# OpenMatchmaking/microservice-matchmaking

Measured on NVIDIA H100. Metric: matches/sec, higher is better.
Workload: dtype int32/u64

## Files before the change

### microservice-matchmaking_b200/csrc/mm_common.cuh

```cuda
#pragma once
#include <cuda_runtime.h>
#include <stdint.h>

#include "../../include/mm_engine.h"

namespace mm {

constexpr int kBlock = 512;
constexpr uint32_t kTile = 2048;
constexpr uint32_t kMaxRows = 2048;
constexpr uint32_t kMaxStages = 4;
constexpr uint32_t kTileBytes = kTile * (8 + 2);
constexpr uint32_t kMaxSegs = MM_MAX_GROUPS * MM_MAX_MODES;
constexpr uint32_t kChunkHist = 256;
constexpr uint32_t kFastBins = 255;
constexpr uint64_t kEmptyKey = 0xFFFFFFFFFFFFFFFFull;
constexpr uint64_t kTombKey = 0xFFFFFFFFFFFFFFFEull;
constexpr uint64_t kFreeVal = 0xFFFFFFFFFFFFFFFFull;
constexpr uint64_t kPending = 0x8000000000000000ull;
constexpr uint32_t kGenMask = 0x7FFFFFFFu;

struct PoolView {
  uint64_t* id;
  int32_t* rating;
  uint8_t* mode;
  uint8_t* tsize;
  uint32_t* ts;
  uint16_t* bin;
  uint32_t* seq;
};
struct PoolMeta {
  uint32_t* fill;
  uint32_t* chunk_tab;
  uint32_t* bump;
  uint32_t* tot;
  uint32_t* chist;
  uint32_t max_ch;
};
// ... 252 lines not shown
```

### microservice-matchmaking_b200/csrc/mm_engine.cu

```cuda
#include <cuda_runtime.h>

#include <algorithm>
#include <cstdio>
#include <cstdlib>
#include <cstring>
#include <mutex>
#include <new>
#include <vector>

#include "mm_kernels.cuh"
#include "mm_stats.cuh"

using namespace mm;

namespace {

struct Pool {
  PoolView v{};
  PoolMeta m{};
  uint32_t n = 0;
};

struct Table {
  unsigned long long* kv = nullptr;
// ... 38 lines not shown
  Pool pool[2];
  int cur = 0;
  uint32_t gen = 1;
  uint32_t seq_next = 0;
  Pool snap;
  uint32_t snap_gen = 0, snap_seq = 0;
  bool has_snap = false;

  bool use_active = true, dense_ids = false;
  uint64_t hcap = 0;
  Table tab[2];
  int tcur = 0;
  uint64_t n_active = 0, n_tomb = 0;

  uint32_t R = 0;
  uint32_t helpers = 0;
  int rows_per_sm = 2;
  int rank_impl = 3;
  uint32_t place_stages = 0;
  int fused_ok = 0;
  int tick_impl = 1;
  size_t tick_smem = 0;
  uint32_t *d_M = nullptr, *d_P = nullptr;
  uint32_t *d_outbase = nullptr, *d_binlim = nullptr;
  uint16_t* d_bin_key = nullptr;
  int32_t max_spread = -1;
  SegInfo* d_seg = nullptr;
  uint32_t* d_left_bits = nullptr;
  uint64_t* d_members = nullptr;
  uint32_t* d_members32 = nullptr;
  uint32_t* d_members32_alt = nullptr;
  mm_lobby_hdr* d_hdr_alt = nullptr;
  uint32_t* d_src_idx = nullptr;
  mm_lobby_hdr* d_hdr = nullptr;
  uint32_t* d_emit_seq = nullptr;
  uint32_t max_lobbies = 0;
  uint32_t* d_rescnt = nullptr;
  TickCtr* d_ctr2 = nullptr;
  TickCtr* d_ctr = nullptr;
  int ctr_idx = 0;
  TickCtr* h_ctr = nullptr;

  uint32_t enq_cap = 0;
  uint64_t *d_in_id = nullptr, *d_hslot = nullptr;
  int32_t* d_in_rating = nullptr;
  uint8_t *d_in_mode = nullptr, *d_code = nullptr;
// ... 237 lines not shown
  CK(cudaMemcpy(e->d_lut, lut.data(), e->KR * 2, cudaMemcpyHostToDevice));
  CK(cudaMemcpy(e->d_grp_lut, grp.data(), e->KR, cudaMemcpyHostToDevice));
  CK(cudaMemcpy(e->d_mode_tsize, tsz.data(), MM_MAX_MODES, cudaMemcpyHostToDevice));
  CK(cudaMemcpy(e->d_seg_bin_lo, seg_lo.data(), (e->n_segs + 1) * 4, cudaMemcpyHostToDevice));
  CK(cudaMemcpy(e->d_seg_L, seg_L.data(), e->n_segs * 4, cudaMemcpyHostToDevice));
  return MM_OK;
}

BinMap bin_map(const mm_engine* e) {
  BinMap b{};
  b.lut = e->d_lut; b.key_lo = e->key_lo; b.KR = e->KR; b.stride = e->stride; b.K = e->K;
  return b;
}

int alloc_tick_scratch(mm_engine* e) {
  uint32_t total = (uint32_t)e->n_sms * (uint32_t)e->rows_per_sm;
  if (total > kMaxRows) total = kMaxRows;
  e->helpers = total >= 64 ? 4u : (total > 1 ? 1u : 0u);
  e->R = total - e->helpers;
  if (e->d_M) { cudaFree(e->d_M); cudaFree(e->d_P); cudaFree(e->d_rescnt); }
  CK(cudaMalloc(&e->d_M, (size_t)(e->R + 1) * e->Kp * 4));
  CK(cudaMalloc(&e->d_P, (size_t)(e->R + 1) * e->Kp * 4));
  CK(cudaMalloc(&e->d_rescnt, (size_t)(e->R + 1) * 4));
  return MM_OK;
}

int ensure_enq_scratch(mm_engine* e, uint32_t n) {
  if (n <= e->enq_cap) return MM_OK;
  cudaFree(e->d_in_id); cudaFree(e->d_hslot); cudaFree(e->d_in_rating); cudaFree(e->d_in_mode);
  cudaFree(e->d_code); cudaFree(e->d_in_ts); cudaFree(e->d_blocksum); cudaFree(e->d_part); cudaFree(e->d_in_key);
  cudaFree(e->d_in_handle);
  e->enq_cap = 0;
  const size_t c = (size_t)n + 64;
  CK(cudaMalloc(&e->d_in_id, c * 8));
  CK(cudaMalloc(&e->d_hslot, c * 8));
  CK(cudaMalloc(&e->d_in_rating, c * 4));
  CK(cudaMalloc(&e->d_in_mode, c));
  CK(cudaMalloc(&e->d_code, c));
  CK(cudaMalloc(&e->d_part, c * 2));
  CK(cudaMalloc(&e->d_in_key, c * 2));
  CK(cudaMalloc(&e->d_in_handle, c * 4));
  CK(cudaMalloc(&e->d_in_ts, c * 4));
  CK(cudaMalloc(&e->d_blocksum, (std::min<size_t>(c, kEnqChunkDev) / 256 + 2) * 4));
  e->enq_cap = n;
  return MM_OK;
}
// ... 80 lines not shown

TailArgs tail_args(mm_engine* e) {
  TailArgs t{};
  t.Kp = e->Kp; t.K = e->K; t.n_segs = e->n_segs; t.max_spread = e->max_spread; t.layout = tail_layout(e);
  t.tot = e->pool[e->cur].m.tot; t.seg_bin_lo = e->d_seg_bin_lo; t.seg_L = e->d_seg_L; t.bin_seg = e->d_bin_seg;
  t.n_cut = e->n_cut; t.part_cut = e->d_part_cut; t.cut_lp_lo = e->d_cut_lp_lo;
  t.bin_key = e->d_bin_key; t.outbase = e->d_outbase; t.binlim = e->d_binlim; t.seg = e->d_seg; t.ctr = e->d_ctr;
  t.fill = e->pool[e->cur].m.fill;
  t.dst = e->pool[e->cur ^ 1].m;
  return t;
}
uint32_t tick_rows(const mm_engine* e) {
  const uint64_t tiles = (uint64_t)e->pool[e->cur].n / kTile + e->n_segs;
  const uint32_t total = e->R + e->helpers;
  const uint32_t want = std::min(32u, std::max(e->helpers, (total * 14 / 100 + e->min_L - 1) / e->min_L));
  return (uint32_t)std::min<uint64_t>(total - want, std::max<uint64_t>(1, (tiles + 1) / 2));
}

PlaceArgs place_args(mm_engine* e, bool want_seq) {
  const Pool& p = e->pool[e->cur];
  PlaceArgs a{};
  a.bins16 = p.v.bin; a.ids = p.v.id; a.meta = p.m;
  a.K = e->K; a.Kp = e->Kp; a.R = tick_rows(e); a.stages = e->place_stages; a.fast_ok = e->rank_impl == 3; a.max_nb = e->max_nb;
  a.seg_bin_lo = e->d_seg_bin_lo; a.bin_seg = e->d_bin_seg; a.M = e->d_M; a.P = e->d_P;
  a.outbase = e->d_outbase; a.binlim = e->d_binlim; a.members = e->d_members;
  a.src_idx = want_seq ? e->d_src_idx : nullptr;
  a.left_bits = e->d_left_bits; a.rescnt = e->d_rescnt; a.ctr = e->d_ctr;
  return a;
}
uint32_t next_gen(const mm_engine* e) { return e->gen >= kGenMask ? 1u : e->gen + 1; }
EpiArgs epi_args(mm_engine* e, bool want_seq, bool headers) {
  EpiArgs a{};
  a.src = e->pool[e->cur].v; a.dst = e->pool[e->cur ^ 1].v;
  a.src_meta = e->pool[e->cur].m; a.dst_meta = e->pool[e->cur ^ 1].m;
  a.R = tick_rows(e); a.new_gen = next_gen(e); a.n_segs = e->n_segs; a.n_groups = e->cfg.n_groups; a.Kp = e->Kp;
  a.write_headers = headers ? 1u : 0u;
  a.rescnt = e->d_rescnt; a.left_bits = e->d_left_bits; a.act = act_view(e); a.seg = e->d_seg; a.seg_L = e->d_seg_L; a.part_cut = e->d_part_cut;
  a.seg_bin_lo = e->d_seg_bin_lo;
  a.hdr = e->d_hdr; a.src_idx = want_seq ? e->d_src_idx : nullptr; a.emit_seq = want_seq ? e->d_emit_seq : nullptr;
  a.ctr = e->d_ctr;
  return a;
}

int tick_phase_a(mm_engine* e) {
  const Pool& p = e->pool[e->cur];
  CK(cudaMemsetAsync(e->d_ctr, 0, sizeof(TickCtr), e->stream));
  CK(cudaEventRecord(e->ev[0], e->stream));
  const uint32_t rows = tick_rows(e);
  k_hist<512><<<rows, 512, hist_smem_bytes(e->max_nb), e->stream>>>(p.v.bin, p.m, e->n_segs, rows, e->Kp, e->max_nb, e->d_seg_bin_lo, e->d_M);
  CK(cudaEventRecord(e->ev[1], e->stream));
  k_colscan<<<(e->K + 31) / 32 + 1, kScanBlock, colscan_smem(e), e->stream>>>(rows, e->d_M, e->d_P, tail_args(e));
  CK(cudaGetLastError());
  return MM_OK;
}

int tick_phase_b(mm_engine* e, bool want_seq) {
  CK(cudaEventRecord(e->ev[2], e->stream));
  const uint32_t rows = tick_rows(e);
  k_place<512><<<rows, 512, place_smem_bytes(e->max_nb, e->place_stages), e->stream>>>(place_args(e, want_seq),
                                                                                  e->pool[e->cur].m.fill, e->n_segs);
  CK(cudaEventRecord(e->ev[3], e->stream));
  if (e->pool[e->cur ^ 1].m.chist)
    CK(cudaMemsetAsync(e->pool[e->cur ^ 1].m.chist, 0, (size_t)e->n_chunks * kChunkHist * 4, e->stream));
  k_epilogue<512><<<std::max<uint32_t>(1, std::min<uint32_t>((uint32_t)e->n_sms, 2 * rows)), 512, 0, e->stream>>>(epi_args(e, want_seq, true));
  CK(cudaGetLastError());
  CK(cudaEventRecord(e->ev[4], e->stream));
  CK(cudaMemcpyAsync(e->h_ctr, e->d_ctr, sizeof(TickCtr), cudaMemcpyDeviceToHost, e->stream));
  CK(cudaStreamSynchronize(e->stream));
  return MM_OK;
}

bool use_fused(const mm_engine* e) { return e->tick_impl == 1 && e->fused_ok; }
// ... 18 lines not shown
  CK(cudaEventRecord(e->ev[4], e->stream));
  CK(cudaMemcpyAsync(e->h_ctr, e->d_ctr, sizeof(TickCtr), cudaMemcpyDeviceToHost, e->stream));
  CK(cudaStreamSynchronize(e->stream));
  return MM_OK;
}

int tick_commit(mm_engine* e, uint32_t n, mm_tick_stats* stats) {
  const TickCtr& c = *e->h_ctr;
  mm_tick_stats st{};
  st.pool_before = n; st.n_lobbies = c.n_lobbies; st.n_matched = c.n_matched; st.n_residual = c.n_resid;
  st.n_dead = c.n_dead; st.n_launches = 4;
  float ms = 0;
  CK(cudaEventElapsedTime(&ms, e->ev[0], e->ev[4]));
  st.device_us = ms * 1000.f;
  if (e->last_fused) {
    st.n_launches = 1;
    st.hist_us = (float)(c.t[1] - c.t[0]) * 1e-3f;
    st.scan_us = (float)(c.t[2] - c.t[1]) * 1e-3f;
    st.place_us = (float)(c.t[3] - c.t[2]) * 1e-3f;
    st.epilogue_us = (float)(c.t[6] - c.t[3]) * 1e-3f;
    if (std::getenv("MM_TRACE")) {
      const double us = 1e3 / ((double)e->clock_khz * tick_rows(e));
      std::fprintf(stderr, "[mm] t0=0 rows_p1_done=%.1f tail_done=%.1f bar1=%.1f place_start=%.1f rows_place_done=%.1f bar2=%.1f end=%.1f us"
                   " | place stall/row hand full empty loop: h0 %.1f %.1f %.1f %.1f h1 %.1f %.1f %.1f %.1f us\n",
                   (c.t[8] - c.t[0]) * 1e-3, (c.t[5] - c.t[0]) * 1e-3, (c.t[1] - c.t[0]) * 1e-3, (c.t[2] - c.t[0]) * 1e-3,
                   (c.t[10] - c.t[0]) * 1e-3, (c.t[3] - c.t[0]) * 1e-3, (c.t[6] - c.t[0]) * 1e-3,
                   c.stall[0][0] * us, c.stall[0][1] * us, c.stall[0][2] * us, c.stall[0][3] * us,
                   c.stall[1][0] * us, c.stall[1][1] * us, c.stall[1][2] * us, c.stall[1][3] * us);
    }
  } else {
    CK(cudaEventElapsedTime(&ms, e->ev[0], e->ev[1]));
    st.hist_us = ms * 1000.f;
    CK(cudaEventElapsedTime(&ms, e->ev[1], e->ev[2]));
    st.scan_us = ms * 1000.f;
    CK(cudaEventElapsedTime(&ms, e->ev[2], e->ev[3]));
    st.place_us = ms * 1000.f;
    CK(cudaEventElapsedTime(&ms, e->ev[3], e->ev[4]));
    st.epilogue_us = ms * 1000.f;
  }
  e->gen = next_gen(e);
  e->cur ^= 1;
  e->pool[e->cur].n = c.n_resid;
  e->match_valid = true;
  e->match_n = n;
  e->last = st;
  if (stats) *stats = st;
  if (c.chist_bad) {
    std::snprintf(e->last_err, sizeof(e->last_err), "%u placement tiles disagree with their chunk histograms", c.chist_bad);
    return MM_E_STATE;
  }
  return MM_OK;
// ... 122 lines not shown
  e->cfg = *cfg;
  e->device = cfg->device;
  e->capacity = cfg->capacity;
  e->use_active = !(cfg->flags & MM_F_NO_DEDUPE);
  e->dense_ids = e->use_active && (cfg->flags & MM_F_DENSE_IDS);
  auto bail = [&](int code) { mm_destroy(e); return code; };
  if (cudaSetDevice(e->device) != cudaSuccess) return bail(MM_E_CUDA);
  cudaDeviceProp prop{};
  if (cudaGetDeviceProperties(&prop, e->device) != cudaSuccess) return bail(MM_E_CUDA);
  e->n_sms = prop.multiProcessorCount;
  if (cudaDeviceGetAttribute(&e->clock_khz, cudaDevAttrClockRate, e->device) != cudaSuccess) return bail(MM_E_CUDA);
  e->smem_optin = prop.sharedMemPerBlockOptin;
  e->smem_sm = prop.sharedMemPerMultiprocessor;
  if (cudaStreamCreateWithFlags(&e->stream, cudaStreamNonBlocking) != cudaSuccess) return bail(MM_E_CUDA);
  if (cudaStreamCreateWithFlags(&e->d2h_stream, cudaStreamNonBlocking) != cudaSuccess) return bail(MM_E_CUDA);
  if (cudaStreamCreateWithFlags(&e->copy_stream, cudaStreamNonBlocking) != cudaSuccess ||
      cudaEventCreateWithFlags(&e->ev_copy, cudaEventDisableTiming) != cudaSuccess)
    return bail(MM_E_CUDA);
  for (auto& ev : e->ev)
    if (cudaEventCreate(&ev) != cudaSuccess) return bail(MM_E_CUDA);
  if ((rc = build_tables(e))) return bail(rc);
  {
    const size_t static_smem = sizeof(Geo) + 512;
    const uint32_t st_max = 2;
    for (uint32_t st = st_max; st >= 2 && !e->place_stages; --st)
      if (2 * (place_smem_bytes(e->max_nb, st) + static_smem + 1024) <= e->smem_sm) { e->place_stages = st; e->rows_per_sm = 2; }
    for (uint32_t st = kMaxStages; st >= 1 && !e->place_stages; --st)
      if (place_smem_bytes(e->max_nb, st) + static_smem + 1024 <= e->smem_optin) { e->place_stages = st; e->rows_per_sm = 1; }
    if (!e->place_stages || colscan_smem(e) + static_smem + 1024 > e->smem_optin) {
      std::snprintf(e->last_err, sizeof(e->last_err), "key domain too large for shared memory: %u bins", e->Kp);
      return bail(MM_E_ARG);
    }
    bool ok = allow_max_smem(e, k_colscan) == cudaSuccess && allow_max_smem(e, k_hist<512>) == cudaSuccess &&
              allow_max_smem(e, k_place<512>) == cudaSuccess && allow_max_smem(e, k_tick<512>) == cudaSuccess;
    if (!ok) return bail(fail(e, cudaGetLastError(), "cudaFuncSetAttribute"));
  }
  e->n_chunks = (e->capacity + kTile - 1) / kTile + e->n_segs + 2;
  if ((uint64_t)e->n_chunks * e->n_segs * 4 > (8ull << 30)) return bail(MM_E_CAP);
  if ((rc = alloc_pool(e, e->pool[0])) || (rc = alloc_pool(e, e->pool[1]))) return bail(rc);
  if (cudaMalloc(&e->d_left_bits, (pool_slots(e) / 32 + 64) * 4) != cudaSuccess) return bail(MM_E_CUDA);
  if (e->use_active) {
    const uint64_t want = cfg->active_capacity ? cfg->active_capacity : 2ull * cfg->capacity;
    if (e->dense_ids) {
      e->hcap = want;
      for (auto& t : e->tab) t.kv = nullptr;
      if (cudaMalloc(&e->tab[0].kv, e->hcap * 8) != cudaSuccess) return bail(MM_E_CUDA);
    } else {
// ... 27 lines not shown
    int coop = 0, nb = 0;
    cudaDeviceGetAttribute(&coop, cudaDevAttrCooperativeLaunch, e->device);
    if (coop && cudaOccupancyMaxActiveBlocksPerMultiprocessor(&nb, k_tick<512>, 512, sz) == cudaSuccess &&
        (uint32_t)nb * (uint32_t)e->n_sms >= e->R + e->helpers) {
      e->fused_ok = 1;
      e->tick_smem = sz;
    }
    cudaGetLastError();
  }
  if (cudaStreamSynchronize(e->stream) != cudaSuccess) return bail(MM_E_CUDA);
  *out = e;
  return MM_OK;
}

int mm_destroy(mm_engine* e) {
  if (!e) return MM_OK;
  cudaSetDevice(e->device);
  if (e->stream) cudaStreamSynchronize(e->stream);
  if (e->d2h_stream) cudaStreamSynchronize(e->d2h_stream);
  free_pool(e->pool[0]); free_pool(e->pool[1]); free_pool(e->snap); cudaFree(e->d_left_bits);
  for (auto& t : e->tab) cudaFree(t.kv);
  cudaFree(e->d_lut); cudaFree(e->d_grp_lut); cudaFree(e->d_mode_tsize); cudaFree(e->d_seg_bin_lo); cudaFree(e->d_seg_L);
  cudaFree(e->d_part_cut); cudaFree(e->d_cut_lp_lo);
  cudaFree(e->d_M); cudaFree(e->d_P); cudaFree(e->d_outbase); cudaFree(e->d_binlim); cudaFree(e->d_bin_seg);
  cudaFree(e->d_bin_key); cudaFree(e->d_seg); cudaFree(e->d_members); cudaFree(e->d_members32); cudaFree(e->d_members32_alt); cudaFree(e->d_hdr_alt); cudaFree(e->d_src_idx);
  cudaFree(e->d_hdr); cudaFree(e->d_emit_seq); cudaFree(e->d_rescnt); cudaFree(e->d_ctr2); cudaFree(e->d_small);
  cudaFree(e->d_in_id); cudaFree(e->d_hslot); cudaFree(e->d_in_rating); cudaFree(e->d_in_mode); cudaFree(e->d_code);
  cudaFree(e->d_in_ts); cudaFree(e->d_blocksum); cudaFree(e->d_blockhist); cudaFree(e->d_part); cudaFree(e->d_in_key);
  cudaFree(e->d_in_handle); cudaFree(e->d_rej_idx); cudaFree(e->d_rej_code);
  cudaFree(e->d_qstat);
  if (e->h_ctr) cudaFreeHost(e->h_ctr);
  if (e->h_small) cudaFreeHost(e->h_small);
  for (auto& ev : e->ev)
    if (ev) cudaEventDestroy(ev);
  if (e->stream && e->own_stream) cudaStreamDestroy(e->stream);
  for (auto& st : e->stage) { cudaFree(st.handle); cudaFree(st.key); cudaFree(st.ts); if (st.ready) cudaEventDestroy(st.ready); }
  if (e->d2h_stream) cudaStreamDestroy(e->d2h_stream);
  if (e->copy_stream) cudaStreamDestroy(e->copy_stream);
  if (e->ev_copy) cudaEventDestroy(e->ev_copy);
  cudaGetLastError();
  delete e;
  return MM_OK;
}

int mm_set_stream(mm_engine* e, void* s) {
  if (!e) return MM_E_ARG;
  std::lock_guard<std::mutex> lk(e->mu);
// ... 450 lines not shown
```

### microservice-matchmaking_b200/csrc/mm_hist.cuh

```cuda
#pragma once
#include "mm_common.cuh"

namespace mm {

constexpr uint32_t kHistStages = 8;

__host__ __device__ constexpr size_t hist_smem_bytes(uint32_t max_nb) {
  return (size_t)kHistStages * kTile * 2 + 256 + (size_t)((max_nb + 4) & ~3u) * 4 + sizeof(DescCache) + 16;
}

template <int BLOCK>
__device__ __forceinline__ void hist_body(unsigned char* smem_raw, const Geo& g, const uint16_t* __restrict__ bins16,
                                          const PoolMeta meta, uint32_t Kp, uint32_t max_nb,
                                          const uint32_t* __restrict__ seg_bin_lo, uint32_t* __restrict__ M) {
  constexpr uint32_t kBytes = kTile * 2, S = kHistStages, H = S / 2;
  uint16_t* ring = reinterpret_cast<uint16_t*>(smem_raw);
  uint64_t* full = reinterpret_cast<uint64_t*>(smem_raw + (size_t)S * kBytes);
  uint32_t* s_nv = reinterpret_cast<uint32_t*>(smem_raw + (size_t)S * kBytes + 64);
  uint32_t* s_sg = s_nv + S;
  uint32_t* s_b0 = s_sg + S;
  uint32_t* s_b1 = s_b0 + S;
  uint32_t* hist = reinterpret_cast<uint32_t*>(smem_raw + (size_t)S * kBytes + 256);
  DescCache& dc = *reinterpret_cast<DescCache*>(hist + ((max_nb + 4) & ~3u));
  const uint32_t tid = threadIdx.x, row = blockIdx.x;
// ... 54 lines not shown
#pragma unroll
      for (uint32_t q = tid; q < kTile / 8; q += BLOCK) {
        const uint32_t o = q * 8;
        if (o + 8 <= valid) {
          const uint4 v = *reinterpret_cast<const uint4*>(tb + o);
          add(v.x & 0xFFFFu); add(v.x >> 16); add(v.y & 0xFFFFu); add(v.y >> 16);
          add(v.z & 0xFFFFu); add(v.z >> 16); add(v.w & 0xFFFFu); add(v.w >> 16);
        } else {
          for (uint32_t e = o; e < valid; ++e) add(tb[e]);
        }
      }
    }
    __syncthreads();
    if (tid == 0)
      for (uint32_t k = 0; k < H && t0 + S + k < n_tiles; ++k) issue(sb + k, t0 + S + k);
  }
  if (cur_sg != 0xFFFFFFFFu) flush();
  if (tid == 0)
    for (uint32_t s = 0; s < kHistStages; ++s) mbar_inval(&full[s]);
}

template <int BLOCK>
__device__ __forceinline__ void rowsum_body(unsigned char* smem_raw, const Geo& g, const PoolMeta meta, uint32_t Kp,
                                            const uint32_t* __restrict__ seg_bin_lo, uint32_t* __restrict__ M) {
  DescCache& dc = *reinterpret_cast<DescCache*>(smem_raw);
  const uint32_t tid = threadIdx.x, row = blockIdx.x;
  const uint32_t s0 = row * g.tpr < g.NT ? row * g.tpr : g.NT;
  const uint32_t s1 = s0 + g.tpr < g.NT ? s0 + g.tpr : g.NT;
  uint32_t* mrow = M + (size_t)row * Kp;
  uint32_t cur_sg = 0xFFFFFFFFu, acc = 0;
  for (uint32_t tb = s0; tb < s1; tb += kDescCap) {
    __syncthreads();
    desc_fill<BLOCK>(dc, g, meta, tb, s1);
    __syncthreads();
    const uint32_t nt = s1 - tb < kDescCap ? s1 - tb : kDescCap;
    constexpr uint32_t U = 8;
    for (uint32_t t0 = 0; t0 < nt; t0 += U) {
      uint32_t v[U];
#pragma unroll
      for (uint32_t u = 0; u < U; ++u)
        v[u] = (t0 + u < nt && tid < kChunkHist) ? __ldcg(&meta.chist[(size_t)dc.phys[t0 + u] * kChunkHist + tid]) : 0u;
#pragma unroll
      for (uint32_t u = 0; u < U; ++u) {
        if (t0 + u >= nt) break;
        const uint32_t sg = dc.nvsg[t0 + u] >> 16;
        if (sg != cur_sg) {
          if (cur_sg != 0xFFFFFFFFu) {
            const uint32_t b0 = seg_bin_lo[cur_sg], nb = seg_bin_lo[cur_sg + 1] - b0;
            if (tid < nb) mrow[b0 + tid] = acc;
          }
          cur_sg = sg; acc = 0;
        }
        acc += v[u];
      }
    }
  }
  if (cur_sg != 0xFFFFFFFFu) {
    const uint32_t b0 = seg_bin_lo[cur_sg], nb = seg_bin_lo[cur_sg + 1] - b0;
    if (tid < nb) mrow[b0 + tid] = acc;
  }
  __syncthreads();
}

}
```

### microservice-matchmaking_b200/csrc/mm_kernels.cuh

```cuda
#pragma once
#include "mm_common.cuh"
#include "mm_hist.cuh"
#include "mm_scan.cuh"
#include "mm_place.cuh"
#include "mm_epilogue.cuh"
#include "mm_active.cuh"

namespace mm {

template <int BLOCK>
__global__ void __launch_bounds__(BLOCK, 2)
    k_hist(const uint16_t* __restrict__ bins16, const PoolMeta meta, uint32_t n_segs, uint32_t R, uint32_t Kp, uint32_t max_nb,
           const uint32_t* __restrict__ seg_bin_lo, uint32_t* __restrict__ M) {
  extern __shared__ __align__(128) unsigned char smem_raw[];
  __shared__ Geo geo;
  __shared__ uint32_t s_gtmp[33];
  geo_build<BLOCK>(geo, meta.fill, n_segs, R, s_gtmp);
  if (meta.chist) rowsum_body<BLOCK>(smem_raw, geo, meta, Kp, seg_bin_lo, M);
  else hist_body<BLOCK>(smem_raw, geo, bins16, meta, Kp, max_nb, seg_bin_lo, M);
}

struct TickArgs {
  PoolView src;
  uint32_t R;
  uint32_t* M;
  uint32_t* P;
  TailArgs tail;
  PlaceArgs place;
  EpiArgs epi;
  TickCtr* next_ctr;
};

template <int BLOCK>
__global__ void __launch_bounds__(BLOCK, 2) k_tick(const TickArgs a) {
  static_assert(BLOCK == kScanBlock, "the column-scan phase is written for 512-thread CTAs");
  extern __shared__ __align__(128) unsigned char smem_raw[];
  __shared__ Geo geo;
  __shared__ uint32_t s_gtmp[33];
  uint32_t* scratch = reinterpret_cast<uint32_t*>(smem_raw);
  const unsigned int G = gridDim.x;
  const uint32_t R = a.R, Kp = a.tail.Kp, K = a.tail.K;
// ... 5 lines not shown
    if (blockIdx.x == 0 && threadIdx.x == 0) {
      unsigned long long t;
      asm volatile("mov.u64 %0, %%globaltimer;" : "=l"(t));
      ctr->t[k] = t;
    }
  };
  stamp(0);
  const bool tail_cta = blockIdx.x == G - 1;
  auto run_tail = [&]() {
    colscan_tail_body(scratch, a.tail);
    if (threadIdx.x == 0) {
      unsigned long long t;
      asm volatile("mov.u64 %0, %%globaltimer;" : "=l"(t));
      ctr->t[5] = t;
    }
  };
  const bool tail_first = tail_cta && !is_row;
  if (tail_first) {
    run_tail();
    grid_arrive(&ctr->gbar);
  }
  geo_build<BLOCK>(geo, a.place.meta.fill, a.tail.n_segs, R, s_gtmp);
  if (is_row) {
    if (a.place.meta.chist) rowsum_body<BLOCK>(smem_raw, geo, a.place.meta, Kp, a.tail.seg_bin_lo, a.M);
    else hist_body<BLOCK>(smem_raw, geo, a.src.bin, a.place.meta, Kp, a.place.max_nb, a.tail.seg_bin_lo, a.M);
  }
  if (tail_cta && is_row) run_tail();
  if (threadIdx.x == 0) { unsigned long long tm; asm volatile("mov.u64 %0, %%globaltimer;" : "=l"(tm)); if (is_row) atomicMax(&ctr->t[8], tm); }
  bar += G;
  if (tail_first) grid_wait(&ctr->gbar, bar); else grid_barrier(&ctr->gbar, bar);
  stamp(1);
  if (geo_use_colscan(geo)) {
    for (uint32_t grp = blockIdx.x; grp < (K + 31) / 32; grp += G) colscan_cols_body(scratch, geo, grp, Kp, K, a.tail.bin_seg, a.M, a.P);
    grid_barrier(&ctr->gbar, (bar += G));
  }
  stamp(2);
  if (is_row) place_body<BLOCK>(smem_raw, geo, a.place);
  if (threadIdx.x == 0 && is_row) { unsigned long long tm; asm volatile("mov.u64 %0, %%globaltimer;" : "=l"(tm)); atomicMax(&ctr->t[10], tm); }
  if (a.epi.dst_meta.chist && (!is_row || n_helpers == 0)) {
    const uint32_t part = n_helpers ? helper : blockIdx.x, nparts = n_helpers ? n_helpers : G;
    const size_t words = (size_t)__ldcg(a.epi.dst_meta.bump) * kChunkHist;
    for (size_t i = (size_t)part * BLOCK + threadIdx.x; i < words; i += (size_t)nparts * BLOCK) a.epi.dst_meta.chist[i] = 0;
  }
  if (is_row && !a.epi.write_headers) headers_claimed<BLOCK>(scratch, a.epi, &ctr->hdr_next);
  grid_barrier(&ctr->gbar, (bar += G));
  stamp(3);
  epilogue_body<BLOCK>(scratch, geo, a.epi, &ctr->t[7]);
// ... 17 lines not shown
```

### microservice-matchmaking_b200/csrc/mm_place.cuh

```cuda
#pragma once
#include "mm_common.cuh"

namespace mm {

constexpr uint32_t kHeadSlots = 4096;
constexpr uint32_t NW16 = 16;
constexpr uint32_t kPlaceUnionBytes = NW16 * 256 * 4 + NW16 * 256 * 2 + 1024 + kTile * 4;

__host__ __device__ constexpr uint32_t place_cnt_cap(uint32_t max_nb) { return (max_nb > 1024u ? max_nb : 1024u); }
constexpr uint32_t kHalfWarps = 8;
constexpr uint32_t kHalfBytes = kHalfWarps * 256 * 4 + kHalfWarps * 256 * 2 + 256 * 4 + kTile * 4;
constexpr uint32_t kHalvesHdr = 288;
__host__ __device__ constexpr size_t place_smem_whole(uint32_t max_nb, uint32_t stages) {
  return (size_t)stages * kTileBytes + 128 + (size_t)((place_cnt_cap(max_nb) + 3) & ~3u) * 4 + kPlaceUnionBytes + sizeof(DescCache) + 16;
}
__host__ __device__ constexpr size_t place_smem_halves(uint32_t max_nb, uint32_t stages) {
  return (size_t)stages * (kTileBytes + kChunkHist * 4) + kHalvesHdr + (size_t)((place_cnt_cap(max_nb) + 3) & ~3u) * 4 +
         2 * kHalfBytes + sizeof(DescCache) + 16;
}
__host__ __device__ constexpr size_t place_smem_bytes(uint32_t max_nb, uint32_t stages) {
  return max_nb <= kFastBins && place_smem_halves(max_nb, stages) > place_smem_whole(max_nb, stages)
             ? place_smem_halves(max_nb, stages)
             : place_smem_whole(max_nb, stages);
}

struct PlaceArgs {
  const uint16_t* bins16;
  const uint64_t* ids;
  PoolMeta meta;
  uint32_t K, Kp, R, stages, fast_ok, max_nb;
  const uint32_t* seg_bin_lo;
  const uint16_t* bin_seg;
  const uint32_t* M;
  const uint32_t* P;
  const uint32_t* outbase;
  const uint32_t* binlim;
  uint64_t* members;
  uint32_t* src_idx;
  uint32_t* left_bits;
  uint32_t* rescnt;
  TickCtr* ctr;
};

template <int BLOCK>
__device__ __forceinline__ void place_halves(unsigned char* smem_raw, const Geo& g, const PlaceArgs a) {
  static_assert(BLOCK == 512 && kTile == 2048, "tile arrangement is written for 2 x 256 threads x 8 players");
  constexpr int J = 8;
  const uint32_t S = a.stages;
  uint64_t* ring_ids = reinterpret_cast<uint64_t*>(smem_raw);
  uint16_t* ring_bins = reinterpret_cast<uint16_t*>(smem_raw + (size_t)S * kTile * 8);
  uint32_t* ring_hist = reinterpret_cast<uint32_t*>(smem_raw + (size_t)S * kTileBytes);
  unsigned char* hdr = smem_raw + (size_t)S * (kTileBytes + kChunkHist * 4);
  uint64_t* full = reinterpret_cast<uint64_t*>(hdr);
  uint64_t* empty = full + kMaxStages;
  uint64_t* hand = empty + kMaxStages;
  uint32_t* s_nv = reinterpret_cast<uint32_t*>(hand + 1);
  uint32_t* s_b0 = s_nv + kMaxStages;
  uint32_t* s_b1 = s_b0 + kMaxStages;
  uint32_t* s_sg = s_b1 + kMaxStages;
  uint32_t* s_misc = s_sg + kMaxStages;
  uint32_t* s_wt = s_misc + 8;
  uint32_t* s_ck = s_wt + 16;
  uint32_t* cnt = reinterpret_cast<uint32_t*>(hdr + kHalvesHdr);
  const uint32_t cnt_cap = place_cnt_cap(a.max_nb);
  unsigned char* halves = reinterpret_cast<unsigned char*>(cnt + ((cnt_cap + 3) & ~3u));
  DescCache& dc = *reinterpret_cast<DescCache*>(halves + 2 * kHalfBytes);

  const uint32_t tid = threadIdx.x, lane = tid & 31, h = tid >> 8, ht = tid & 255, hw = ht >> 5;
  const uint32_t lt_mask = (1u << lane) - 1u;
  uint32_t* wmask = reinterpret_cast<uint32_t*>(halves + h * kHalfBytes);
  uint16_t* wcnt = reinterpret_cast<uint16_t*>(wmask + kHalfWarps * 256);
  uint32_t* lgd = reinterpret_cast<uint32_t*>(wcnt + kHalfWarps * 256);
  uint32_t* spd = lgd + 256;
  const uint32_t row = blockIdx.x;
  const uint64_t pol_in = policy_evict_first();

  const uint32_t s0 = row * g.tpr < g.NT ? row * g.tpr : g.NT;
  const uint32_t s1 = s0 + g.tpr < g.NT ? s0 + g.tpr : g.NT;
  const uint32_t n_tiles = s1 - s0;

  auto issue = [&](uint32_t stage, uint32_t t) {
    uint32_t phys, nvsg;
    if (t < kDescCap) { phys = dc.phys[t]; nvsg = dc.nvsg[t]; }
    else { const TileDesc d = geo_tile(g, a.meta, s0 + t); phys = d.phys; nvsg = d.nvalid | (d.seg << 16); }
    s_nv[stage] = nvsg & 0xFFFFu;
    s_sg[stage] = nvsg >> 16;
    s_b0[stage] = a.seg_bin_lo[nvsg >> 16];
    s_b1[stage] = a.seg_bin_lo[(nvsg >> 16) + 1];
    mbar_expect_tx(&full[stage], kTileBytes + kChunkHist * 4);
    tma_load_1d(ring_ids + (size_t)stage * kTile, a.ids + (size_t)phys * kTile, kTile * 8, &full[stage], pol_in);
    tma_load_1d(ring_bins + (size_t)stage * kTile, a.bins16 + (size_t)phys * kTile, kTile * 2, &full[stage], pol_in);
    tma_load_1d(ring_hist + (size_t)stage * kChunkHist, a.meta.chist + (size_t)phys * kChunkHist, kChunkHist * 4,
                &full[stage], pol_in);
  };

  if (tid == 0) {
    for (uint32_t s = 0; s < S; ++s) { mbar_init(&full[s], 1); mbar_init(&empty[s], 256); }
    mbar_init(hand, 256);
    mbar_fence_init();
    for (uint32_t i = 0; i < 8; ++i) { s_misc[i] = 0; s_ck[i] = 0; }
  }
  fence_proxy_async();
  desc_fill<BLOCK>(dc, g, a.meta, s0, s1);
  for (uint32_t i = tid; i < 2 * (kHalfWarps * 256 * 6 / 4); i += BLOCK) {
    const uint32_t hh = i / (kHalfWarps * 256 * 6 / 4), k = i % (kHalfWarps * 256 * 6 / 4);
    reinterpret_cast<uint32_t*>(halves + hh * kHalfBytes)[k] = 0;
  }
  __syncthreads();
  if (tid == 0)
    for (uint32_t t = 0; t < S && t < n_tiles; ++t) issue(t, t);

  uint32_t nleft = 0;
  const uint32_t row_p_last = n_tiles ? geo_seg_of(g, s1 - 1) : 0u;
  const bool scanned = geo_use_colscan(g);
  uint32_t* ck = s_ck + 4 * h;
  if (ht == 0) ck[3] = (uint32_t)clock();
  for (uint32_t t = h; t < n_tiles; t += 2) {
    const uint32_t st = t % S, parity = (t / S) & 1u;
    const uint32_t vbase = (s0 + t) * kTile;
    const uint16_t* tb = ring_bins + (size_t)st * kTile;
    const uint64_t* ti = ring_ids + (size_t)st * kTile;
    const uint32_t ck0 = (uint32_t)clock();
    if (t) mbar_wait(hand, (t - 1) & 1u);
    const uint32_t ck1 = (uint32_t)clock();
    mbar_wait(&full[st], parity);
    if (ht == 0) { ck[0] += ck1 - ck0; ck[1] += (uint32_t)clock() - ck1; }
    const uint32_t valid = s_nv[st];
    const uint32_t bin0 = s_b0[st], nb = s_b1[st] - bin0;
    const uint32_t d = ht;
    const uint32_t ch = d < nb ? ring_hist[st * kChunkHist + d] : 0u;
    const uint32_t lim = ch ? __ldcg(&a.binlim[bin0 + d]) : 0u;
    uint32_t wb = s_misc[1], we = s_misc[2];
    if (bin0 < wb || bin0 + nb > we) {
      wb = bin0; we = bin0 + nb;
      for (uint32_t p = s_sg[st] + 1; p <= row_p_last; ++p) {
        const uint32_t e = a.seg_bin_lo[p + 1];
        if (e - wb > cnt_cap) break;
        we = e;
      }
      for (uint32_t i = wb + ht; i < we; i += 256) {
        uint32_t rlo = 0, rhi = 0, v = 0;
        if (geo_rows_of(g, a.bin_seg[i], rlo, rhi) && row >= rlo && row <= rhi) {
          uint32_t pre = 0;
          if (scanned) pre = __ldcg(&a.P[(size_t)row * a.Kp + i]);
          else
            for (uint32_t r = rlo; r < row; r += 8) {
              uint32_t v8[8];
#pragma unroll
              for (uint32_t u = 0; u < 8; ++u) v8[u] = r + u < row ? __ldcg(&a.M[(size_t)(r + u) * a.Kp + i]) : 0u;
#pragma unroll
              for (uint32_t u = 0; u < 8; ++u) pre += v8[u];
            }
          v = __ldcg(&a.outbase[i]) + pre;
        }
        cnt[i - wb] = v;
      }
      bar_sync_half(h);
      if (ht == 0) { s_misc[1] = wb; s_misc[2] = we; }
    }
    uint32_t base = 0;
    if (d < nb) { base = cnt[bin0 - wb + d]; cnt[bin0 - wb + d] = base + ch; }
    mbar_arrive(hand);

    uint32_t incl = ch;
#pragma unroll
    for (int off = 1; off < 32; off <<= 1) {
      const uint32_t u = __shfl_up_sync(0xFFFFFFFFu, incl, off);
      if (lane >= (uint32_t)off) incl += u;
    }
    if (lane == 31) s_wt[h * 8 + hw] = incl;

    uint32_t pk[J];
    {
      uint32_t* wm = wmask + hw * 256;
      uint16_t* wc = wcnt + hw * 256;
      uint32_t dg[J];
#pragma unroll
      for (int j = 0; j < J; ++j) {
        const uint32_t pos = hw * (32 * J) + j * 32 + lane;
        const uint32_t dd = (uint32_t)tb[pos] - bin0;
        dg[j] = (pos < valid && dd < nb) ? dd : nb;
      }
      const uint32_t lbit = 1u << lane;
      if (nb > 16) {
#pragma unroll
// ... 67 lines not shown
            if (e >> 31) matched = slot < __ldcg(&a.binlim[bin0 + dj]);
            if (matched && a.src_idx) a.src_idx[slot] = vbase + pos;
          }
          spd[lpos] = pos | ((matched ? dj : 255u) << 11);
          if (!matched) lmask |= 1u << j;
        }
      }
    }
    {
      uint32_t mine = 0, all = 0;
      if (tf & 1u) {
#pragma unroll
        for (int j = 0; j < J; ++j) {
          const uint32_t wv = __ballot_sync(0xFFFFFFFFu, (lmask >> j) & 1u);
          if (lane == (uint32_t)j) mine = wv;
          all += __popc(wv);
        }
      }
      if (lane < (uint32_t)J) a.left_bits[(vbase >> 5) + hw * J + lane] = mine;
      if (lane == 0) nleft += all;
    }
    __syncwarp();
    reinterpret_cast<uint4*>(wcnt + hw * 256)[lane] = make_uint4(0, 0, 0, 0);
    bar_sync_half(h);
    if (ht == 0) {
      s_misc[3 + h] = 0;
      if (tf & 2u) atomicAdd(&a.ctr->chist_bad, 1u);
    }
    if (!(tf & 2u)) {
#pragma unroll
      for (int i = 0; i < J; ++i) {
        const uint32_t k = i * 256 + ht;
        if (k < n_live) {
          const uint32_t v = spd[k], dk = v >> 11;
          if (dk != 255u) a.members[(lgd[dk] + k) & 0x7FFFFFFFu] = ti[v & 0x7FFu];
        }
      }
    }
    mbar_arrive(&empty[st]);
    if (ht == 0 && t + S < n_tiles) {
      const uint32_t ck2 = (uint32_t)clock();
      mbar_wait(&empty[st], parity);
      ck[2] += (uint32_t)clock() - ck2;
      issue(st, t + S);
    }
  }
  if (ht == 0) {
    ck[3] = (uint32_t)clock() - ck[3];
    for (uint32_t k = 0; k < 4; ++k) atomicAdd(&a.ctr->stall[h][k], (unsigned long long)ck[k]);
  }

  if (lane == 0 && nleft) atomicAdd(&s_misc[0], nleft);
  __syncthreads();
  if (tid == 0) {
    a.rescnt[row] = s_misc[0];
    for (uint32_t s = 0; s < S; ++s) { mbar_inval(&full[s]); mbar_inval(&empty[s]); }
    mbar_inval(hand);
  }
}

template <int BLOCK>
__device__ __forceinline__ void place_body(unsigned char* smem_raw, const Geo& g, const PlaceArgs a) {
  static_assert(BLOCK == 512 && kTile == 2048, "tile arrangement is written for 512 threads x 4 players");
  if (a.meta.chist && a.fast_ok) {
    place_halves<BLOCK>(smem_raw, g, a);
    return;
  }
  constexpr int J = kTile / BLOCK;
  constexpr int NW = BLOCK / 32;
  const uint32_t stages = a.stages, K = a.K, Kp = a.Kp;
  uint64_t* ring_ids = reinterpret_cast<uint64_t*>(smem_raw);
  uint16_t* ring_bins = reinterpret_cast<uint16_t*>(smem_raw + (size_t)stages * kTile * 8);
  uint64_t* full = reinterpret_cast<uint64_t*>(smem_raw + (size_t)stages * kTileBytes);
  uint32_t* s_nv = reinterpret_cast<uint32_t*>(smem_raw + (size_t)stages * kTileBytes + 32);
  uint32_t* s_sg = s_nv + kMaxStages;
  uint32_t* s_b0 = s_sg + kMaxStages;
  uint32_t* s_b1 = s_b0 + kMaxStages;
  uint32_t* s_misc = s_b1 + kMaxStages;
  uint32_t* cnt = reinterpret_cast<uint32_t*>(smem_raw + (size_t)stages * kTileBytes + 128);
  const uint32_t cnt_cap = place_cnt_cap(a.max_nb);
  unsigned char* uni = reinterpret_cast<unsigned char*>(cnt + ((cnt_cap + 3) & ~3u));
  DescCache& dc = *reinterpret_cast<DescCache*>(uni + kPlaceUnionBytes);
  uint32_t* head = reinterpret_cast<uint32_t*>(uni);
  uint32_t* node = head + kHeadSlots;
  uint16_t* nbin = reinterpret_cast<uint16_t*>(node + kTile);
  uint32_t* wmask = reinterpret_cast<uint32_t*>(uni);
  uint16_t* wcnt = reinterpret_cast<uint16_t*>(wmask + NW * 256);
  uint32_t* wcnt32 = reinterpret_cast<uint32_t*>(wcnt);
  uint32_t* lgd = wcnt32 + NW * 128;
  uint32_t* spd = lgd + 256;
// ... 357 lines not shown
```

Measured before the change: 6.409 billion.

## Precompute per-tile bin prefixes in hist pass and decouple place halves

The row-sum pass now writes a per-tile word packing each bin's running prefix within its segment together with the tile count. The place kernel TMA-loads this word instead of the raw chunk histogram. That lets each half compute its base offsets independently, so the serial 'hand' barrier between the two halves goes away and tiles are handed out dynamically through a shared counter. The per-bin window of base offsets is built once up front, the default place pipeline depth rises from 2 to 3 stages, and a fallback path is taken when a row has too many tiles or bins. In exchange there is extra global write traffic in the hist pass, another scratch buffer, and a spin-wait on stage tags.

```diff
diff --git a/microservice-matchmaking_b200/csrc/mm_common.cuh b/microservice-matchmaking_b200/csrc/mm_common.cuh
--- a/microservice-matchmaking_b200/csrc/mm_common.cuh
+++ b/microservice-matchmaking_b200/csrc/mm_common.cuh
@@ -14,6 +14,8 @@
 constexpr uint32_t kMaxSegs = MM_MAX_GROUPS * MM_MAX_MODES;
 constexpr uint32_t kChunkHist = 256;
 constexpr uint32_t kFastBins = 255;
+constexpr uint32_t kTilePreMaxTiles = 512;
+__host__ __device__ constexpr uint32_t tile_pre_word(uint32_t prefix, uint32_t count) { return prefix << 12 | count; }
 constexpr uint64_t kEmptyKey = 0xFFFFFFFFFFFFFFFFull;
 constexpr uint64_t kTombKey = 0xFFFFFFFFFFFFFFFEull;
 constexpr uint64_t kFreeVal = 0xFFFFFFFFFFFFFFFFull;
diff --git a/microservice-matchmaking_b200/csrc/mm_engine.cu b/microservice-matchmaking_b200/csrc/mm_engine.cu
--- a/microservice-matchmaking_b200/csrc/mm_engine.cu
+++ b/microservice-matchmaking_b200/csrc/mm_engine.cu
@@ -84,6 +84,7 @@
   int tick_impl = 1;
   size_t tick_smem = 0;
   uint32_t *d_M = nullptr, *d_P = nullptr;
+  uint32_t* d_tpre = nullptr;
   uint32_t *d_outbase = nullptr, *d_binlim = nullptr;
   uint16_t* d_bin_key = nullptr;
   int32_t max_spread = -1;
@@ -367,6 +368,8 @@
   CK(cudaMalloc(&e->d_M, (size_t)(e->R + 1) * e->Kp * 4));
   CK(cudaMalloc(&e->d_P, (size_t)(e->R + 1) * e->Kp * 4));
   CK(cudaMalloc(&e->d_rescnt, (size_t)(e->R + 1) * 4));
+  if (e->max_nb <= kFastBins && !e->d_tpre)
+    CK(cudaMalloc(&e->d_tpre, (size_t)e->n_chunks * kChunkHist * 4));
   return MM_OK;
 }
 
@@ -493,7 +496,7 @@
   PlaceArgs a{};
   a.bins16 = p.v.bin; a.ids = p.v.id; a.meta = p.m;
   a.K = e->K; a.Kp = e->Kp; a.R = tick_rows(e); a.stages = e->place_stages; a.fast_ok = e->rank_impl == 3; a.max_nb = e->max_nb;
-  a.seg_bin_lo = e->d_seg_bin_lo; a.bin_seg = e->d_bin_seg; a.M = e->d_M; a.P = e->d_P;
+  a.seg_bin_lo = e->d_seg_bin_lo; a.bin_seg = e->d_bin_seg; a.M = e->d_M; a.P = e->d_P; a.tpre = e->d_tpre;
   a.outbase = e->d_outbase; a.binlim = e->d_binlim; a.members = e->d_members;
   a.src_idx = want_seq ? e->d_src_idx : nullptr;
   a.left_bits = e->d_left_bits; a.rescnt = e->d_rescnt; a.ctr = e->d_ctr;
@@ -518,7 +521,8 @@
   CK(cudaMemsetAsync(e->d_ctr, 0, sizeof(TickCtr), e->stream));
   CK(cudaEventRecord(e->ev[0], e->stream));
   const uint32_t rows = tick_rows(e);
-  k_hist<512><<<rows, 512, hist_smem_bytes(e->max_nb), e->stream>>>(p.v.bin, p.m, e->n_segs, rows, e->Kp, e->max_nb, e->d_seg_bin_lo, e->d_M);
+  k_hist<512><<<rows, 512, hist_smem_bytes(e->max_nb), e->stream>>>(p.v.bin, p.m, e->n_segs, rows, e->Kp, e->max_nb,
+                                                                   e->d_seg_bin_lo, e->d_M, e->d_tpre);
   CK(cudaEventRecord(e->ev[1], e->stream));
   k_colscan<<<(e->K + 31) / 32 + 1, kScanBlock, colscan_smem(e), e->stream>>>(rows, e->d_M, e->d_P, tail_args(e));
   CK(cudaGetLastError());
@@ -583,11 +587,11 @@
     if (std::getenv("MM_TRACE")) {
       const double us = 1e3 / ((double)e->clock_khz * tick_rows(e));
       std::fprintf(stderr, "[mm] t0=0 rows_p1_done=%.1f tail_done=%.1f bar1=%.1f place_start=%.1f rows_place_done=%.1f bar2=%.1f end=%.1f us"
-                   " | place stall/row hand full empty loop: h0 %.1f %.1f %.1f %.1f h1 %.1f %.1f %.1f %.1f us\n",
+                   " | place stall/row window %.1f, full empty loop: h0 %.1f %.1f %.1f h1 %.1f %.1f %.1f us\n",
                    (c.t[8] - c.t[0]) * 1e-3, (c.t[5] - c.t[0]) * 1e-3, (c.t[1] - c.t[0]) * 1e-3, (c.t[2] - c.t[0]) * 1e-3,
                    (c.t[10] - c.t[0]) * 1e-3, (c.t[3] - c.t[0]) * 1e-3, (c.t[6] - c.t[0]) * 1e-3,
                    c.stall[0][0] * us, c.stall[0][1] * us, c.stall[0][2] * us, c.stall[0][3] * us,
-                   c.stall[1][0] * us, c.stall[1][1] * us, c.stall[1][2] * us, c.stall[1][3] * us);
+                   c.stall[1][1] * us, c.stall[1][2] * us, c.stall[1][3] * us);
     }
   } else {
     CK(cudaEventElapsedTime(&ms, e->ev[0], e->ev[1]));
@@ -756,7 +760,7 @@
   if ((rc = build_tables(e))) return bail(rc);
   {
     const size_t static_smem = sizeof(Geo) + 512;
-    const uint32_t st_max = 2;
+    const uint32_t st_max = 3;
     for (uint32_t st = st_max; st >= 2 && !e->place_stages; --st)
       if (2 * (place_smem_bytes(e->max_nb, st) + static_smem + 1024) <= e->smem_sm) { e->place_stages = st; e->rows_per_sm = 2; }
     for (uint32_t st = kMaxStages; st >= 1 && !e->place_stages; --st)
@@ -830,7 +834,7 @@
   for (auto& t : e->tab) cudaFree(t.kv);
   cudaFree(e->d_lut); cudaFree(e->d_grp_lut); cudaFree(e->d_mode_tsize); cudaFree(e->d_seg_bin_lo); cudaFree(e->d_seg_L);
   cudaFree(e->d_part_cut); cudaFree(e->d_cut_lp_lo);
-  cudaFree(e->d_M); cudaFree(e->d_P); cudaFree(e->d_outbase); cudaFree(e->d_binlim); cudaFree(e->d_bin_seg);
+  cudaFree(e->d_M); cudaFree(e->d_P); cudaFree(e->d_tpre); cudaFree(e->d_outbase); cudaFree(e->d_binlim); cudaFree(e->d_bin_seg);
   cudaFree(e->d_bin_key); cudaFree(e->d_seg); cudaFree(e->d_members); cudaFree(e->d_members32); cudaFree(e->d_members32_alt); cudaFree(e->d_hdr_alt); cudaFree(e->d_src_idx);
   cudaFree(e->d_hdr); cudaFree(e->d_emit_seq); cudaFree(e->d_rescnt); cudaFree(e->d_ctr2); cudaFree(e->d_small);
   cudaFree(e->d_in_id); cudaFree(e->d_hslot); cudaFree(e->d_in_rating); cudaFree(e->d_in_mode); cudaFree(e->d_code);
diff --git a/microservice-matchmaking_b200/csrc/mm_hist.cuh b/microservice-matchmaking_b200/csrc/mm_hist.cuh
--- a/microservice-matchmaking_b200/csrc/mm_hist.cuh
+++ b/microservice-matchmaking_b200/csrc/mm_hist.cuh
@@ -100,12 +100,14 @@
 
 template <int BLOCK>
 __device__ __forceinline__ void rowsum_body(unsigned char* smem_raw, const Geo& g, const PoolMeta meta, uint32_t Kp,
-                                            const uint32_t* __restrict__ seg_bin_lo, uint32_t* __restrict__ M) {
+                                            const uint32_t* __restrict__ seg_bin_lo, uint32_t* __restrict__ M,
+                                            uint32_t* __restrict__ tpre) {
   DescCache& dc = *reinterpret_cast<DescCache*>(smem_raw);
   const uint32_t tid = threadIdx.x, row = blockIdx.x;
   const uint32_t s0 = row * g.tpr < g.NT ? row * g.tpr : g.NT;
   const uint32_t s1 = s0 + g.tpr < g.NT ? s0 + g.tpr : g.NT;
   uint32_t* mrow = M + (size_t)row * Kp;
+  uint32_t* pre = tpre && s1 - s0 <= kTilePreMaxTiles && tid < kChunkHist ? tpre + tid : nullptr;
   uint32_t cur_sg = 0xFFFFFFFFu, acc = 0;
   for (uint32_t tb = s0; tb < s1; tb += kDescCap) {
     __syncthreads();
@@ -129,6 +131,7 @@
           }
           cur_sg = sg; acc = 0;
         }
+        if (pre) pre[(size_t)(tb + t0 + u) * kChunkHist] = tile_pre_word(acc, v[u]);
         acc += v[u];
       }
     }
@@ -137,6 +140,7 @@
     const uint32_t b0 = seg_bin_lo[cur_sg], nb = seg_bin_lo[cur_sg + 1] - b0;
     if (tid < nb) mrow[b0 + tid] = acc;
   }
+  if (pre) asm volatile("fence.proxy.async.global;" ::: "memory");
   __syncthreads();
 }
 
diff --git a/microservice-matchmaking_b200/csrc/mm_kernels.cuh b/microservice-matchmaking_b200/csrc/mm_kernels.cuh
--- a/microservice-matchmaking_b200/csrc/mm_kernels.cuh
+++ b/microservice-matchmaking_b200/csrc/mm_kernels.cuh
@@ -11,12 +11,12 @@
 template <int BLOCK>
 __global__ void __launch_bounds__(BLOCK, 2)
     k_hist(const uint16_t* __restrict__ bins16, const PoolMeta meta, uint32_t n_segs, uint32_t R, uint32_t Kp, uint32_t max_nb,
-           const uint32_t* __restrict__ seg_bin_lo, uint32_t* __restrict__ M) {
+           const uint32_t* __restrict__ seg_bin_lo, uint32_t* __restrict__ M, uint32_t* __restrict__ tpre) {
   extern __shared__ __align__(128) unsigned char smem_raw[];
   __shared__ Geo geo;
   __shared__ uint32_t s_gtmp[33];
   geo_build<BLOCK>(geo, meta.fill, n_segs, R, s_gtmp);
-  if (meta.chist) rowsum_body<BLOCK>(smem_raw, geo, meta, Kp, seg_bin_lo, M);
+  if (meta.chist) rowsum_body<BLOCK>(smem_raw, geo, meta, Kp, seg_bin_lo, M, tpre);
   else hist_body<BLOCK>(smem_raw, geo, bins16, meta, Kp, max_nb, seg_bin_lo, M);
 }
 
@@ -68,7 +68,7 @@
   }
   geo_build<BLOCK>(geo, a.place.meta.fill, a.tail.n_segs, R, s_gtmp);
   if (is_row) {
-    if (a.place.meta.chist) rowsum_body<BLOCK>(smem_raw, geo, a.place.meta, Kp, a.tail.seg_bin_lo, a.M);
+    if (a.place.meta.chist) rowsum_body<BLOCK>(smem_raw, geo, a.place.meta, Kp, a.tail.seg_bin_lo, a.M, a.place.tpre);
     else hist_body<BLOCK>(smem_raw, geo, a.src.bin, a.place.meta, Kp, a.place.max_nb, a.tail.seg_bin_lo, a.M);
   }
   if (tail_cta && is_row) run_tail();
diff --git a/microservice-matchmaking_b200/csrc/mm_place.cuh b/microservice-matchmaking_b200/csrc/mm_place.cuh
--- a/microservice-matchmaking_b200/csrc/mm_place.cuh
+++ b/microservice-matchmaking_b200/csrc/mm_place.cuh
@@ -33,6 +33,7 @@
   const uint16_t* bin_seg;
   const uint32_t* M;
   const uint32_t* P;
+  uint32_t* tpre;
   const uint32_t* outbase;
   const uint32_t* binlim;
   uint64_t* members;
@@ -43,27 +44,34 @@
 };
 
 template <int BLOCK>
-__device__ __forceinline__ void place_halves(unsigned char* smem_raw, const Geo& g, const PlaceArgs a) {
+__device__ __forceinline__ bool place_halves(unsigned char* smem_raw, const Geo& g, const PlaceArgs a) {
   static_assert(BLOCK == 512 && kTile == 2048, "tile arrangement is written for 2 x 256 threads x 8 players");
   constexpr int J = 8;
   const uint32_t S = a.stages;
+  const uint32_t row = blockIdx.x;
+  const uint32_t s0 = row * g.tpr < g.NT ? row * g.tpr : g.NT;
+  const uint32_t s1 = s0 + g.tpr < g.NT ? s0 + g.tpr : g.NT;
+  const uint32_t n_tiles = s1 - s0;
+  const uint32_t cnt_cap = place_cnt_cap(a.max_nb);
+  const uint32_t wb = n_tiles ? a.seg_bin_lo[geo_seg_of(g, s0)] : 0u;
+  const uint32_t we = n_tiles ? a.seg_bin_lo[geo_seg_of(g, s1 - 1) + 1] : 0u;
+  if (n_tiles > kTilePreMaxTiles || we - wb > cnt_cap) return false;
+
   uint64_t* ring_ids = reinterpret_cast<uint64_t*>(smem_raw);
   uint16_t* ring_bins = reinterpret_cast<uint16_t*>(smem_raw + (size_t)S * kTile * 8);
-  uint32_t* ring_hist = reinterpret_cast<uint32_t*>(smem_raw + (size_t)S * kTileBytes);
+  uint32_t* ring_pre = reinterpret_cast<uint32_t*>(smem_raw + (size_t)S * kTileBytes);
   unsigned char* hdr = smem_raw + (size_t)S * (kTileBytes + kChunkHist * 4);
   uint64_t* full = reinterpret_cast<uint64_t*>(hdr);
   uint64_t* empty = full + kMaxStages;
-  uint64_t* hand = empty + kMaxStages;
-  uint32_t* s_nv = reinterpret_cast<uint32_t*>(hand + 1);
+  uint32_t* s_nv = reinterpret_cast<uint32_t*>(empty + kMaxStages);
   uint32_t* s_b0 = s_nv + kMaxStages;
   uint32_t* s_b1 = s_b0 + kMaxStages;
-  uint32_t* s_sg = s_b1 + kMaxStages;
-  uint32_t* s_misc = s_sg + kMaxStages;
+  uint32_t* s_tag = s_b1 + kMaxStages;
+  uint32_t* s_misc = s_tag + kMaxStages;
   uint32_t* s_wt = s_misc + 8;
   uint32_t* s_ck = s_wt + 16;
-  uint32_t* cnt = reinterpret_cast<uint32_t*>(hdr + kHalvesHdr);
-  const uint32_t cnt_cap = place_cnt_cap(a.max_nb);
-  unsigned char* halves = reinterpret_cast<unsigned char*>(cnt + ((cnt_cap + 3) & ~3u));
+  uint32_t* win = reinterpret_cast<uint32_t*>(hdr + kHalvesHdr);
+  unsigned char* halves = reinterpret_cast<unsigned char*>(win + ((cnt_cap + 3) & ~3u));
   DescCache& dc = *reinterpret_cast<DescCache*>(halves + 2 * kHalfBytes);
 
   const uint32_t tid = threadIdx.x, lane = tid & 31, h = tid >> 8, ht = tid & 255, hw = ht >> 5;
@@ -72,33 +80,28 @@
   uint16_t* wcnt = reinterpret_cast<uint16_t*>(wmask + kHalfWarps * 256);
   uint32_t* lgd = reinterpret_cast<uint32_t*>(wcnt + kHalfWarps * 256);
   uint32_t* spd = lgd + 256;
-  const uint32_t row = blockIdx.x;
   const uint64_t pol_in = policy_evict_first();
-
-  const uint32_t s0 = row * g.tpr < g.NT ? row * g.tpr : g.NT;
-  const uint32_t s1 = s0 + g.tpr < g.NT ? s0 + g.tpr : g.NT;
-  const uint32_t n_tiles = s1 - s0;
 
   auto issue = [&](uint32_t stage, uint32_t t) {
     uint32_t phys, nvsg;
     if (t < kDescCap) { phys = dc.phys[t]; nvsg = dc.nvsg[t]; }
     else { const TileDesc d = geo_tile(g, a.meta, s0 + t); phys = d.phys; nvsg = d.nvalid | (d.seg << 16); }
     s_nv[stage] = nvsg & 0xFFFFu;
-    s_sg[stage] = nvsg >> 16;
     s_b0[stage] = a.seg_bin_lo[nvsg >> 16];
     s_b1[stage] = a.seg_bin_lo[(nvsg >> 16) + 1];
+    *reinterpret_cast<volatile uint32_t*>(&s_tag[stage]) = t;
     mbar_expect_tx(&full[stage], kTileBytes + kChunkHist * 4);
     tma_load_1d(ring_ids + (size_t)stage * kTile, a.ids + (size_t)phys * kTile, kTile * 8, &full[stage], pol_in);
     tma_load_1d(ring_bins + (size_t)stage * kTile, a.bins16 + (size_t)phys * kTile, kTile * 2, &full[stage], pol_in);
-    tma_load_1d(ring_hist + (size_t)stage * kChunkHist, a.meta.chist + (size_t)phys * kChunkHist, kChunkHist * 4,
+    tma_load_1d(ring_pre + (size_t)stage * kChunkHist, a.tpre + (size_t)(s0 + t) * kChunkHist, kChunkHist * 4,
                 &full[stage], pol_in);
   };
 
   if (tid == 0) {
-    for (uint32_t s = 0; s < S; ++s) { mbar_init(&full[s], 1); mbar_init(&empty[s], 256); }
-    mbar_init(hand, 256);
+    for (uint32_t s = 0; s < S; ++s) { mbar_init(&full[s], 1); mbar_init(&empty[s], 256); s_tag[s] = ~0u; }
     mbar_fence_init();
     for (uint32_t i = 0; i < 8; ++i) { s_misc[i] = 0; s_ck[i] = 0; }
+    s_misc[1] = 2;
   }
   fence_proxy_async();
   desc_fill<BLOCK>(dc, g, a.meta, s0, s1);
@@ -109,58 +112,49 @@
   __syncthreads();
   if (tid == 0)
     for (uint32_t t = 0; t < S && t < n_tiles; ++t) issue(t, t);
+  {
+    const uint32_t ckw = (uint32_t)clock();
+    const bool scanned = geo_use_colscan(g);
+    for (uint32_t i = wb + tid; i < we; i += BLOCK) {
+      uint32_t rlo = 0, rhi = 0, v = 0;
+      if (geo_rows_of(g, a.bin_seg[i], rlo, rhi) && row >= rlo && row <= rhi) {
+        uint32_t pre = 0;
+        if (scanned) pre = __ldcg(&a.P[(size_t)row * a.Kp + i]);
+        else
+          for (uint32_t r = rlo; r < row; r += 8) {
+            uint32_t v8[8];
+#pragma unroll
+            for (uint32_t u = 0; u < 8; ++u) v8[u] = r + u < row ? __ldcg(&a.M[(size_t)(r + u) * a.Kp + i]) : 0u;
+#pragma unroll
+            for (uint32_t u = 0; u < 8; ++u) pre += v8[u];
+          }
+        v = __ldcg(&a.outbase[i]) + pre;
+      }
+      win[i - wb] = v;
+    }
+    __syncthreads();
+    if (tid == 0) s_ck[0] = (uint32_t)clock() - ckw;
+  }
 
   uint32_t nleft = 0;
-  const uint32_t row_p_last = n_tiles ? geo_seg_of(g, s1 - 1) : 0u;
-  const bool scanned = geo_use_colscan(g);
   uint32_t* ck = s_ck + 4 * h;
   if (ht == 0) ck[3] = (uint32_t)clock();
-  for (uint32_t t = h; t < n_tiles; t += 2) {
+  for (uint32_t t = h; t < n_tiles;) {
     const uint32_t st = t % S, parity = (t / S) & 1u;
     const uint32_t vbase = (s0 + t) * kTile;
     const uint16_t* tb = ring_bins + (size_t)st * kTile;
     const uint64_t* ti = ring_ids + (size_t)st * kTile;
-    const uint32_t ck0 = (uint32_t)clock();
-    if (t) mbar_wait(hand, (t - 1) & 1u);
     const uint32_t ck1 = (uint32_t)clock();
+    while (*reinterpret_cast<volatile uint32_t*>(&s_tag[st]) != t) __nanosleep(32);
     mbar_wait(&full[st], parity);
-    if (ht == 0) { ck[0] += ck1 - ck0; ck[1] += (uint32_t)clock() - ck1; }
+    if (ht == 0) ck[1] += (uint32_t)clock() - ck1;
     const uint32_t valid = s_nv[st];
     const uint32_t bin0 = s_b0[st], nb = s_b1[st] - bin0;
     const uint32_t d = ht;
-    const uint32_t ch = d < nb ? ring_hist[st * kChunkHist + d] : 0u;
+    const uint32_t pw = d < nb ? ring_pre[st * kChunkHist + d] : 0u;
+    const uint32_t ch = pw & 0xFFFu;
+    const uint32_t base = d < nb ? win[bin0 - wb + d] + (pw >> 12) : 0u;
     const uint32_t lim = ch ? __ldcg(&a.binlim[bin0 + d]) : 0u;
-    uint32_t wb = s_misc[1], we = s_misc[2];
-    if (bin0 < wb || bin0 + nb > we) {
-      wb = bin0; we = bin0 + nb;
-      for (uint32_t p = s_sg[st] + 1; p <= row_p_last; ++p) {
-        const uint32_t e = a.seg_bin_lo[p + 1];
-        if (e - wb > cnt_cap) break;
-        we = e;
-      }
-      for (uint32_t i = wb + ht; i < we; i += 256) {
-        uint32_t rlo = 0, rhi = 0, v = 0;
-        if (geo_rows_of(g, a.bin_seg[i], rlo, rhi) && row >= rlo && row <= rhi) {
-          uint32_t pre = 0;
-          if (scanned) pre = __ldcg(&a.P[(size_t)row * a.Kp + i]);
-          else
-            for (uint32_t r = rlo; r < row; r += 8) {
-              uint32_t v8[8];
-#pragma unroll
-              for (uint32_t u = 0; u < 8; ++u) v8[u] = r + u < row ? __ldcg(&a.M[(size_t)(r + u) * a.Kp + i]) : 0u;
-#pragma unroll
-              for (uint32_t u = 0; u < 8; ++u) pre += v8[u];
-            }
-          v = __ldcg(&a.outbase[i]) + pre;
-        }
-        cnt[i - wb] = v;
-      }
-      bar_sync_half(h);
-      if (ht == 0) { s_misc[1] = wb; s_misc[2] = we; }
-    }
-    uint32_t base = 0;
-    if (d < nb) { base = cnt[bin0 - wb + d]; cnt[bin0 - wb + d] = base + ch; }
-    mbar_arrive(hand);
 
     uint32_t incl = ch;
 #pragma unroll
@@ -274,7 +268,9 @@
     }
     __syncwarp();
     reinterpret_cast<uint4*>(wcnt + hw * 256)[lane] = make_uint4(0, 0, 0, 0);
+    if (ht == 0) s_misc[5 + h] = atomicAdd(&s_misc[1], 1u);
     bar_sync_half(h);
+    const uint32_t t_next = s_misc[5 + h];
     if (ht == 0) {
       s_misc[3 + h] = 0;
       if (tf & 2u) atomicAdd(&a.ctr->chist_bad, 1u);
@@ -296,6 +292,7 @@
       ck[2] += (uint32_t)clock() - ck2;
       issue(st, t + S);
     }
+    t = t_next;
   }
   if (ht == 0) {
     ck[3] = (uint32_t)clock() - ck[3];
@@ -307,17 +304,14 @@
   if (tid == 0) {
     a.rescnt[row] = s_misc[0];
     for (uint32_t s = 0; s < S; ++s) { mbar_inval(&full[s]); mbar_inval(&empty[s]); }
-    mbar_inval(hand);
-  }
+  }
+  return true;
 }
 
 template <int BLOCK>
 __device__ __forceinline__ void place_body(unsigned char* smem_raw, const Geo& g, const PlaceArgs a) {
   static_assert(BLOCK == 512 && kTile == 2048, "tile arrangement is written for 512 threads x 4 players");
-  if (a.meta.chist && a.fast_ok) {
-    place_halves<BLOCK>(smem_raw, g, a);
-    return;
-  }
+  if (a.meta.chist && a.fast_ok && place_halves<BLOCK>(smem_raw, g, a)) return;
   constexpr int J = kTile / BLOCK;
   constexpr int NW = BLOCK / 32;
   const uint32_t stages = a.stages, K = a.K, Kp = a.Kp;
```

Result: no change. 6.522 billion (median of 6 runs) (+1.8%).
